# jscanvic/Scale-Equivariant-Imaging

Measured on AMD Instinct MI355X. Metric: training images/sec (256x256 crops), proposed-loss deblur, higher is better.
Workload: dtype bf16; 1 GPU; BASELINE configs[1]: deblurring Gaussian_R2 noise=5, proposed loss (SURE + scale-EI), 256x256 pairs cropped to 48 in Loss.forward, ConvolutionalModel hidden=32 scales=5; parameters=645063043, batch_per_gpu=32, global_batch=32, parallelism=dp1

## Files before the change

scale-equivariant-imaging_amd/csrc/gemm_bf16nt.hip:

```cpp
#include "sei_common.h"

namespace {

typedef __attribute__((address_space(3))) void lds_void;
typedef __attribute__((address_space(1))) const void glb_void;

constexpr int BK = 64;
constexpr int ROW_BYTES = 128;
constexpr int NWAVES = 8, NT = 512;

__device__ __attribute__((aligned(16))) unsigned short g_zero_chunk[8] = {0, 0, 0, 0, 0, 0, 0, 0};

struct NtArgs {
    const unsigned short *A, *B;
    float *D32;
    unsigned short *D16;
    int M, N, K, lda, ldb;
    int epilogue;
    const float *bias, *R1, *R2;
    unsigned short *D2_16;
    int splitk, k_per_split;
    int tiles_m, tiles_n;
    int tiles_per_xcd, band;
    const unsigned short *A2, *B2;
// ... 52 lines not shown

__device__ __forceinline__ void stage_piece_rmajor(const unsigned short *__restrict__ G,
                                                   const unsigned short *__restrict__ G2, int k_seg, int ld, int o0,
                                                   int o_lim, int k0, int k_lim, char *lds_tile, int q, int lane) {
    const int row = 4 * q + (lane >> 4);
    const int ch = (lane & 15) ^ swz_rmajor(row);
    const int k = k0 + row, o = o0 + 8 * ch;
    const unsigned short *rowp = k < k_seg ? G + (size_t)k * ld : G2 + (size_t)(k - k_seg) * ld;
    const unsigned short *src = (k < k_lim && o < o_lim) ? rowp + o : g_zero_chunk;
    dma16_lane(src, lds_tile + q * 1024);
}
__device__ __forceinline__ void stage_tile_rmajor(const unsigned short *__restrict__ G,
                                                  const unsigned short *__restrict__ G2, int k_seg, int ld, int o0,
                                                  int o_lim, int k0, int k_lim, char *lds_tile, int wave, int lane) {
#pragma unroll
    for (int q0 = 0; q0 < 16; q0 += NWAVES)
        stage_piece_rmajor(G, G2, k_seg, ld, o0, o_lim, k0, k_lim, lds_tile, q0 + wave, lane);
}

__device__ __forceinline__ bf16x8 frag_rmajor(const char *tile, int s, int lane, int c0) {
    const int g = lane >> 4, i16 = lane & 15, q = i16 >> 2, p = i16 & 3;
    const int col0 = c0 + 16 * (g & 1);
    const int row = 16 * s + 8 * (g >> 1) + q;
    const int chunk = (col0 >> 3) + (p >> 1);
    auto addr = [&](int r) {
        return (__attribute__((address_space(3))) v4s *)(tile + 256 * r + 16 * (chunk ^ swz_rmajor(r)) + 8 * (p & 1));
    };
    const v4s lo = __builtin_amdgcn_ds_read_tr16_b64_v4i16(addr(row));
    const v4s hi = __builtin_amdgcn_ds_read_tr16_b64_v4i16(addr(row + 4));
    const v8s both = __builtin_shufflevector(lo, hi, 0, 1, 2, 3, 4, 5, 6, 7);
    return __builtin_bit_cast(bf16x8, both);
}

template <int TM, int TN, int WM, int WN, int NSTAGE>
constexpr bool patch_fits() {
    return (NSTAGE * (32 * TM * WM + 32 * TN * WN) * ROW_BYTES) / (32 * TN * WN * 4) >= 32 * TM;
}

template <int TM, int TN, int WM, int WN, bool ARM, bool BRM, int NSTAGE = 2, int ROWEPI = 0>
__global__ __launch_bounds__(NT, (NSTAGE == 1 ? 3 : 1)) void gemm_bf16nt_kernel(NtArgs g) {
    static_assert(WM * WN == NWAVES, "8 waves per workgroup");
    constexpr int BM = 32 * TM * WM, BN = 32 * TN * WN;
    static_assert(!ARM || BM == 128, "a reduction-major A tile is 64 x 128");
    static_assert(!BRM || BN % 128 == 0, "a reduction-major B tile is BN/128 images of 64 k-rows x 128 columns");
    constexpr int STAGE = (BM + BN) * ROW_BYTES;
    __shared__ __attribute__((aligned(1024))) char smem[NSTAGE * STAGE];

    const int lane = threadIdx.x & 63;
    const int wave = __builtin_amdgcn_readfirstlane(threadIdx.x >> 6);
    const int wm = wave / WN, wn = wave % WN;
    const int li = lane & 31, lh = lane >> 5;

    int bid = blockIdx.x;
    const unsigned short *Bp = g.B, *B2p = g.B2;
    float *D32p = g.D32;
    if constexpr (ROWEPI == 3) {
        const int per = gridDim.x / g.batch, bt = bid / per;
        bid -= bt * per;
        const ptrdiff_t shift = (ptrdiff_t)g.batch_row[bt] * g.ldb;
        Bp += shift;
        B2p += shift;
        D32p += (size_t)bt * g.batch_ld;
    }
    int zs, ord;
    if (g.tiles_per_xcd == 0) {
        const int ntile = g.tiles_m * g.tiles_n;
        zs = bid / ntile;
        ord = bid - zs * ntile;
    } else {
        const int per_split = 8 * g.tiles_per_xcd;
        zs = bid / per_split;
        bid -= zs * per_split;
        ord = (bid & 7) * g.tiles_per_xcd + (bid >> 3);
        if ((bid >> 3) >= g.tiles_per_xcd || ord >= g.tiles_m * g.tiles_n) return;
    }
    int tm_i, tn_i;
    {
        const int band_tiles = g.tiles_m * g.band;
        const int b = ord / band_tiles, r = ord - b * band_tiles;
        const int width = min(g.band, g.tiles_n - b * g.band);
        tm_i = r / width;
        tn_i = b * g.band + (r - tm_i * width);
    }
    const int m0 = tm_i * BM, n0 = tn_i * BN;
    const int M = g.M, N = g.N, K = g.K;
    const int k_begin = zs * g.k_per_split;
    const int k_end = min(K, k_begin + g.k_per_split);

    f32x16 acc[TM][TN];
#pragma unroll
    for (int i = 0; i < TM; ++i)
#pragma unroll
        for (int j = 0; j < TN; ++j)
#pragma unroll
            for (int r = 0; r < 16; ++r) acc[i][j][r] = 0.f;

    constexpr bool PREFETCH_AUX = false;
    const int epi = g.epilogue;
    const bool lead = zs == 0;
    const bool split = g.splitk > 1;
    const float *aux1p = nullptr, *aux2p = nullptr;
    if (epi == SEI_EPI_BIAS_RES && (!split || lead)) { aux1p = g.R1; aux2p = g.R2; }
    else if (epi == SEI_EPI_BIAS_SCALE_RES) aux1p = g.R2;
    else if (epi == SEI_EPI_MUL_DGELU) aux1p = g.R1;
    else if (epi == SEI_EPI_ACCUM && !split) aux1p = D32p;
    float a1[TM][TN][16], a2[TM][TN][16];
    auto gather_aux = [&](int i, int j) {
        const int col = n0 + wn * (32 * TN) + 32 * j + li;
        const int row_base = m0 + wm * (32 * TM) + 32 * i + 4 * lh;
#pragma unroll
        for (int r = 0; r < 16; ++r) {
            const int row = row_base + (r & 3) + 8 * (r >> 2);
            const bool ok = col < N && row < M;
            const size_t o = (size_t)row * N + col;
            a1[i][j][r] = (ok && aux1p) ? aux1p[o] : 0.f;
            a2[i][j][r] = (ok && aux2p) ? aux2p[o] : 0.f;
        }
    };
    if constexpr (PREFETCH_AUX) {
        if (aux1p) {
#pragma unroll
            for (int i = 0; i < TM; ++i)
#pragma unroll
                for (int j = 0; j < TN; ++j) gather_aux(i, j);
        } else {
#pragma unroll
            for (int i = 0; i < TM; ++i)
#pragma unroll
                for (int j = 0; j < TN; ++j)
#pragma unroll
                    for (int r = 0; r < 16; ++r) a1[i][j][r] = a2[i][j][r] = 0.f;
        }
    }

    constexpr int NPA = ARM ? 2 : (BM + 63) / 64, NPB = BN / 64;
    static_assert(BN % 64 == 0, "whole pieces per wave");
    unsigned off_a[NPA], off_b[NPB];
#pragma unroll
    for (int e = 0; e < NPA; ++e) {
        const int q = wave + NWAVES * e;
        if constexpr (ARM) {
            const int row = 4 * q + (lane >> 4), ch = (lane & 15) ^ swz_rmajor(row);
            off_a[e] = (unsigned)row * (unsigned)g.lda * 2u + 2u * (unsigned)min(8 * ch, M - 8 - m0);
        } else {
            const int row = 8 * q + (lane >> 3), c = (lane & 7) ^ ((row >> 1) & 7);
            off_a[e] = (unsigned)min(row, M - 1 - m0) * (unsigned)g.lda * 2u + 16u * c;
        }
    }
#pragma unroll
    for (int e = 0; e < NPB; ++e) {
        const int q = wave + NWAVES * e;
        if constexpr (BRM) {
            const int im = q >> 4, qq = q & 15;
            const int row = 4 * qq + (lane >> 4), ch = (lane & 15) ^ swz_rmajor(row);
            off_b[e] = (unsigned)row * (unsigned)g.ldb * 2u +
                       2u * (unsigned)max(min(128 * im + 8 * ch, N - 8 - n0), 0);
        } else {
            const int row = 8 * q + (lane >> 3), c = (lane & 7) ^ ((row >> 1) & 7);
            off_b[e] = (unsigned)min(row, N - 1 - n0) * (unsigned)g.ldb * 2u + 16u * c;
        }
    }
    auto rm_base = [&](const unsigned short *X1, const unsigned short *X2, int ld, int o0, int k0) -> const char * {
        if (k0 + BK <= g.k_seg && k0 + BK <= k_end) return reinterpret_cast<const char *>(X1 + (size_t)k0 * ld + o0);
        if (k0 >= g.k_seg && k0 + BK <= k_end) return reinterpret_cast<const char *>(X2 + (size_t)(k0 - g.k_seg) * ld + o0);
        return nullptr;
    };
    auto stage = [&](int k0, char *dst) {
        const char *ab, *bb;
        if constexpr (ARM) ab = rm_base(g.A, g.A2, g.lda, m0, k0);
        else if (g.conv_cin > 0) {
            const int tap = k0 / g.conv_cin;
            ab = reinterpret_cast<const char *>(g.A + ((ptrdiff_t)m0 + g.conv_off[tap]) * (ptrdiff_t)g.lda +
                                                (k0 - tap * g.conv_cin));
        }
        else ab = k0 + BK <= k_end ? reinterpret_cast<const char *>(g.A + (size_t)m0 * g.lda + k0) : nullptr;
        if (ab) {
#pragma unroll
            for (int e = 0; e < NPA; ++e)
                if (ARM || wave + NWAVES * e < BM / 8)
                    dma16_base(ab, off_a[e], dst + (wave + NWAVES * e) * 1024);
        } else {
            if constexpr (ARM) stage_tile_rmajor(g.A, g.A2, g.k_seg, g.lda, m0, M, k0, k_end, dst, wave, lane);
            else stage_tile<BM>(g.A, g.lda, m0, M, k0, k_end, dst, wave, lane);
        }
        if constexpr (BRM) bb = rm_base(Bp, B2p, g.ldb, n0, k0);
        else bb = k0 + BK <= k_end ? reinterpret_cast<const char *>(Bp + (size_t)n0 * g.ldb + k0) : nullptr;
        if (bb) {
#pragma unroll
            for (int e = 0; e < NPB; ++e)
                dma16_base(bb, off_b[e], dst + BM * ROW_BYTES + (wave + NWAVES * e) * 1024);
        } else if constexpr (BRM) {
#pragma unroll
            for (int im = 0; im < BN / 128; ++im)
                stage_tile_rmajor(Bp, B2p, g.k_seg, g.ldb, n0 + 128 * im, N, k0, k_end,
                                  dst + BM * ROW_BYTES + im * 16384, wave, lane);
        } else {
            stage_tile<BN>(Bp, g.ldb, n0, N, k0, k_end, dst + BM * ROW_BYTES, wave, lane);
        }
    };
    const int sw = (li >> 1) & 7;
    const int a_off = (wm * 32 * TM + li) * ROW_BYTES;
    const int b_off = BM * ROW_BYTES + (wn * 32 * TN + li) * ROW_BYTES;

    auto compute = [&](const char *now) {
#pragma unroll
        for (int s = 0; s < BK / 16; ++s) {
            const int pc = ((2 * s + lh) ^ sw) * 16;
            bf16x8 a[TM], b[TN];
#pragma unroll
            for (int i = 0; i < TM; ++i) {
                if constexpr (ARM) a[i] = frag_rmajor(now, s, lane, wm * 32 * TM + 32 * i);
                else a[i] = *reinterpret_cast<const bf16x8 *>(now + a_off + i * 32 * ROW_BYTES + pc);
            }
#pragma unroll
            for (int j = 0; j < TN; ++j) {
                if constexpr (BRM) {
                    const int c0 = wn * 32 * TN + 32 * j;
                    b[j] = frag_rmajor(now + BM * ROW_BYTES + (c0 >> 7) * 16384, s, lane, c0 & 127);
                }
                else b[j] = *reinterpret_cast<const bf16x8 *>(now + b_off + j * 32 * ROW_BYTES + pc);
            }
#pragma unroll
            for (int i = 0; i < TM; ++i)
#pragma unroll
                for (int j = 0; j < TN; ++j)
                    acc[i][j] = __builtin_amdgcn_mfma_f32_32x32x16_bf16(a[i], b[j], acc[i][j], 0, 0, 0);
        }
    };

    if constexpr (NSTAGE == 1) {
        for (int k0 = k_begin; k0 < k_end; k0 += BK) {
            stage(k0, smem);
            asm volatile("s_waitcnt vmcnt(0)" ::: "memory");
            __syncthreads();
            compute(smem);
            __syncthreads();
        }
    } else if constexpr (NSTAGE == 2) {
        stage(k_begin, smem);
        asm volatile("s_waitcnt vmcnt(0)" ::: "memory");
        __syncthreads();
        int cur = 0;
        for (int k0 = k_begin; k0 < k_end; k0 += BK) {
            if (k0 + BK < k_end) stage(k0 + BK, smem + (cur ^ 1) * STAGE);
            compute(smem + cur * STAGE);
            asm volatile("s_waitcnt vmcnt(0)" ::: "memory");
            __syncthreads();
            cur ^= 1;
        }
    } else {
        constexpr int PER = (BM + BN) / 64;
        static_assert((BM + BN) % 64 == 0, "uniform DMA count per wave");
        const int nt = (k_end - k_begin + BK - 1) / BK;
#pragma unroll
        for (int t = 0; t < NSTAGE - 1; ++t)
            if (t < nt) stage(k_begin + t * BK, smem + t * STAGE);
        int slot = 0;
        for (int t = 0; t < nt; ++t) {
            if (t + NSTAGE - 2 < nt) sei_wait_vmcnt<(NSTAGE - 2) * PER>();
            else sei_wait_vmcnt<0>();
            __builtin_amdgcn_s_barrier();
            const int tn = t + NSTAGE - 1;
            if (tn < nt) {
                int ns = slot + NSTAGE - 1;
                if (ns >= NSTAGE) ns -= NSTAGE;
                stage(k_begin + tn * BK, smem + ns * STAGE);
            }
            compute(smem + slot * STAGE);
            if (++slot == NSTAGE) slot = 0;
        }
        sei_wait_vmcnt<0>();
    }

    if constexpr (ROWEPI == 2) {
        static_assert(TM == 2 && TN == 1 && WM == 2 && WN == 4, "the row patch below is laid out for the 128 x 128 tile");
        float *patch = reinterpret_cast<float *>(smem);
#pragma unroll
        for (int h = 0; h < 2; ++h) {
            __builtin_amdgcn_s_barrier();
            if (wm == h) {
#pragma unroll
                for (int i = 0; i < TM; ++i)
#pragma unroll
                    for (int r = 0; r < 16; ++r)
                        patch[(32 * i + 4 * lh + (r & 3) + 8 * (r >> 2)) * 128 + 32 * wn + li] = acc[i][0][r];
            }
            __syncthreads();
#pragma unroll
            for (int k = 0; k < 4; ++k) {
                const int idx = threadIdx.x + NT * k, r = idx >> 5, c4 = idx & 31;
                const int row = m0 + 64 * h + r, col = n0 + 4 * c4;
                if (row >= M || col >= N) continue;
                const float4 v = *reinterpret_cast<const float4 *>(patch + r * 128 + 4 * c4);
                uint2 w;
                w.x = sei_pack2_bf16(v.x, v.y);
                w.y = sei_pack2_bf16(v.z, v.w);
                *reinterpret_cast<uint2 *>(g.D16 + (size_t)row * N + col) = w;
            }
        }
        return;
    }
    if constexpr (ROWEPI == 1) {
        static_assert(TM == 2 && TN == 1 && WM == 2 && WN == 4, "the row patch below is laid out for the 128 x 128 tile");
        const float beta1 = g.adam_h[0], beta2 = g.adam_h[1], eps = g.adam_h[2], wd = g.adam_h[3];
        const float step_size = g.adam_h[4], inv_bc2_sqrt = g.adam_h[5];
        float *patch = reinterpret_cast<float *>(smem);
#pragma unroll
        for (int h = 0; h < 2; ++h) {
            __builtin_amdgcn_s_barrier();
            if (wm == h) {
#pragma unroll
                for (int i = 0; i < TM; ++i)
#pragma unroll
                    for (int r = 0; r < 16; ++r)
                        patch[(32 * i + 4 * lh + (r & 3) + 8 * (r >> 2)) * 128 + 32 * wn + li] = acc[i][0][r];
            }
            __syncthreads();
#pragma unroll 1
          for (int kk = 0; kk < 4; kk += 2) {
            float4 gq[2], pq[2], mq[2], vq[2];
            size_t off[2];
            bool ok[2];
#pragma unroll
            for (int k = 0; k < 2; ++k) {
                const int idx = threadIdx.x + NT * (kk + k), r = idx >> 5, c4 = idx & 31;
                const int row = m0 + 64 * h + r, col = n0 + 4 * c4;
                ok[k] = row < M && col < N;
                off[k] = ok[k] ? (size_t)row * N + col : 0;
                gq[k] = *reinterpret_cast<const float4 *>(patch + r * 128 + 4 * c4);
                pq[k] = nt_load4(g.adam_p + off[k]);
                mq[k] = nt_load4(g.adam_m + off[k]);
                vq[k] = nt_load4(g.adam_v + off[k]);
            }
#pragma unroll
            for (int k = 0; k < 2; ++k) {
                if (!ok[k]) continue;
                float4 o;
                o.x = sei_adam_element(pq[k].x, gq[k].x, mq[k].x, vq[k].x, beta1, beta2, eps, wd, step_size, inv_bc2_sqrt);
                o.y = sei_adam_element(pq[k].y, gq[k].y, mq[k].y, vq[k].y, beta1, beta2, eps, wd, step_size, inv_bc2_sqrt);
                o.z = sei_adam_element(pq[k].z, gq[k].z, mq[k].z, vq[k].z, beta1, beta2, eps, wd, step_size, inv_bc2_sqrt);
                o.w = sei_adam_element(pq[k].w, gq[k].w, mq[k].w, vq[k].w, beta1, beta2, eps, wd, step_size, inv_bc2_sqrt);
                nt_store4(g.adam_m + off[k], mq[k]);
                nt_store4(g.adam_v + off[k], vq[k]);
                nt_store4(g.adam_p + off[k], o);
                if (g.adam_p16) {
                    uint2 w;
                    w.x = sei_pack2_bf16(o.x, o.y);
                    w.y = sei_pack2_bf16(o.z, o.w);
                    u32x2 t;
                    t.x = w.x; t.y = w.y;
                    __builtin_nontemporal_store(t, reinterpret_cast<u32x2 *>(g.adam_p16 + off[k]));
                }
            }
          }
        }
        return;
    }

    if constexpr ((ROWEPI == 4 || ROWEPI == 5) && patch_fits<TM, TN, WM, WN, NSTAGE>()) {
        constexpr int ROWS_WM = 32 * TM;
        constexpr int LDS_ROWS = (NSTAGE * STAGE) / (BN * 4);
        constexpr int GW = LDS_ROWS >= WM * ROWS_WM ? WM : (LDS_ROWS >= 2 * ROWS_WM && WM >= 2 ? 2 : 1);
        static_assert(LDS_ROWS >= ROWS_WM && WM % GW == 0, "one wave row of the tile fits the operand stages");
        constexpr int RP = GW * ROWS_WM, QPR = BN / 4, TOTAL = RP * QPR;
        float *patch = reinterpret_cast<float *>(smem);
        const bool to_bf16_only = g.D16 != nullptr && D32p == nullptr;
#pragma unroll 1
        for (int pass = 0; pass < WM / GW; ++pass) {
            __builtin_amdgcn_s_barrier();
            if (wm / GW == pass) {
#pragma unroll
                for (int i = 0; i < TM; ++i)
#pragma unroll
                    for (int j = 0; j < TN; ++j)
#pragma unroll
                        for (int r = 0; r < 16; ++r)
                            patch[((wm % GW) * ROWS_WM + 32 * i + 4 * lh + (r & 3) + 8 * (r >> 2)) * BN + wn * (32 * TN) +
                                  32 * j + li] = acc[i][j][r];
            }
            __syncthreads();
            constexpr int U = NSTAGE == 1 ? 1 : 2;
#pragma unroll 1
            for (int base = threadIdx.x; base < TOTAL; base += U * NT) {
                float4 v[U], r1[U], r2[U];
                size_t off[U];
                int rowi[U];
                bool ok[U];
#pragma unroll
                for (int u = 0; u < U; ++u) {
                    const int idx = base + u * NT;
                    const int r = idx / QPR, c4 = idx - r * QPR;
                    int row = m0 + pass * RP + r;
                    const int col = n0 + 4 * c4;
                    ok[u] = idx < TOTAL && row < M && col < N;
                    if constexpr (ROWEPI == 5) {
                        const int Wp = g.unpad_W + 2, HWp = (g.unpad_H + 2) * Wp;
                        const int b = row / HWp, rem = row - b * HWp, yy = rem / Wp, xx = rem - yy * Wp;
                        ok[u] = ok[u] && yy >= 1 && yy <= g.unpad_H && xx >= 1 && xx <= g.unpad_W;
                        row = (b * g.unpad_H + yy - 1) * g.unpad_W + xx - 1;
                    }
                    off[u] = ok[u] ? (size_t)row * N + col : 0;
                    rowi[u] = ok[u] ? row : 0;
                    v[u] = *reinterpret_cast<const float4 *>(patch + (idx < TOTAL ? r * BN + 4 * c4 : 0));
                    r1[u] = r2[u] = make_float4(0.f, 0.f, 0.f, 0.f);
                    if (epi == SEI_EPI_BIAS || epi == SEI_EPI_BIAS_GELU || epi == SEI_EPI_BIAS_RES ||
                        epi == SEI_EPI_BIAS_ROWSCALE || epi == SEI_EPI_BIAS_SCALE_RES) {
                        const int cb = ok[u] ? col : 0;
                        float4 b = make_float4(g.bias[cb], g.bias[cb + 1], g.bias[cb + 2], g.bias[cb + 3]);
                        if (epi == SEI_EPI_BIAS_ROWSCALE) {
                            const float sc = g.R1[rowi[u]];
                            b.x *= sc; b.y *= sc; b.z *= sc; b.w *= sc;
                        }
                        v[u].x += b.x; v[u].y += b.y; v[u].z += b.z; v[u].w += b.w;
                    }
                    if (epi == SEI_EPI_BIAS_RES || epi == SEI_EPI_MUL_DGELU)
                        r1[u] = *reinterpret_cast<const float4 *>(g.R1 + off[u]);
                    else if (epi == SEI_EPI_ACCUM) r1[u] = *reinterpret_cast<const float4 *>(D32p + off[u]);
                    if (epi == SEI_EPI_BIAS_SCALE_RES || (epi == SEI_EPI_BIAS_RES && g.R2))
                        r2[u] = *reinterpret_cast<const float4 *>(g.R2 + off[u]);
                }
#pragma unroll
                for (int u = 0; u < U; ++u) {
                    if (!ok[u]) continue;
                    float4 o = v[u];
                    if (epi == SEI_EPI_MUL_DGELU) {
                        if (to_bf16_only) {
                            o.x *= sei_dgelu_bf16out(r1[u].x); o.y *= sei_dgelu_bf16out(r1[u].y);
                            o.z *= sei_dgelu_bf16out(r1[u].z); o.w *= sei_dgelu_bf16out(r1[u].w);
                        } else {
                            o.x *= sei_dgelu(r1[u].x); o.y *= sei_dgelu(r1[u].y);
                            o.z *= sei_dgelu(r1[u].z); o.w *= sei_dgelu(r1[u].w);
                        }
                    } else if (epi == SEI_EPI_BIAS_SCALE_RES) {
                        const float sc = g.R1[rowi[u]];
                        o.x = fmaf(o.x, sc, r2[u].x); o.y = fmaf(o.y, sc, r2[u].y);
                        o.z = fmaf(o.z, sc, r2[u].z); o.w = fmaf(o.w, sc, r2[u].w);
                    } else {
                        if (ROWEPI == 5 && g.unpad_act) {
                            o.x = o.x > 0.f ? o.x : 0.01f * o.x; o.y = o.y > 0.f ? o.y : 0.01f * o.y;
                            o.z = o.z > 0.f ? o.z : 0.01f * o.z; o.w = o.w > 0.f ? o.w : 0.01f * o.w;
                        }
                        o.x += r1[u].x + r2[u].x; o.y += r1[u].y + r2[u].y;
                        o.z += r1[u].z + r2[u].z; o.w += r1[u].w + r2[u].w;
                    }
                    if (epi == SEI_EPI_BIAS_GELU) {
                        uint2 w;
                        w.x = (unsigned)sei_f2bf(sei_gelu_bf16out(o.x)) | ((unsigned)sei_f2bf(sei_gelu_bf16out(o.y)) << 16);
                        w.y = (unsigned)sei_f2bf(sei_gelu_bf16out(o.z)) | ((unsigned)sei_f2bf(sei_gelu_bf16out(o.w)) << 16);
                        *reinterpret_cast<uint2 *>(g.D2_16 + off[u]) = w;
                    }
                    if (D32p) *reinterpret_cast<float4 *>(D32p + off[u]) = o;
                    if (g.D16) {
                        uint2 w;
                        w.x = sei_pack2_bf16(o.x, o.y);
                        w.y = sei_pack2_bf16(o.z, o.w);
                        *reinterpret_cast<uint2 *>(g.D16 + off[u]) = w;
                    }
                }
            }
        }
        return;
    }

#pragma unroll
    for (int i = 0; i < TM; ++i) {
#pragma unroll
        for (int j = 0; j < TN; ++j) {
            const int col = n0 + wn * (32 * TN) + 32 * j + li;
            const bool col_ok = col < N;
            const int row_base = m0 + wm * (32 * TM) + 32 * i + 4 * lh;
            float bias = (col_ok && (!split || lead) &&
                          (epi == SEI_EPI_BIAS || epi == SEI_EPI_BIAS_GELU || epi == SEI_EPI_BIAS_RES ||
                           epi == SEI_EPI_BIAS_ROWSCALE || epi == SEI_EPI_BIAS_SCALE_RES))
                             ? g.bias[col] : 0.f;
            if constexpr (!PREFETCH_AUX) gather_aux(i, j);
            if (epi == SEI_EPI_BIAS_ROWSCALE) {
#pragma unroll
                for (int r = 0; r < 16; ++r) {
                    const int row = row_base + (r & 3) + 8 * (r >> 2);
                    a1[i][j][r] = row < M ? bias * g.R1[row] : 0.f;
                }
                bias = 0.f;
            }
#pragma unroll
            for (int r = 0; r < 16; ++r) {
                const int row = row_base + (r & 3) + 8 * (r >> 2);
                if (!col_ok || row >= M) continue;
                const size_t o = (size_t)row * N + col;
                float v = acc[i][j][r] + bias;
                if (split) {
                    atomicAdd(D32p + o, v + a1[i][j][r] + a2[i][j][r]);
                    continue;
                }
                if (epi == SEI_EPI_MUL_DGELU)
                    v *= (g.D16 && !D32p) ? sei_dgelu_bf16out(a1[i][j][r]) : sei_dgelu(a1[i][j][r]);
                else if (epi == SEI_EPI_BIAS_SCALE_RES) v = fmaf(v, g.R1[row], a1[i][j][r]);
                else v += a1[i][j][r] + a2[i][j][r];
                if (epi == SEI_EPI_BIAS_GELU) g.D2_16[o] = sei_f2bf(sei_gelu_bf16out(v));
                if (D32p) D32p[o] = v;
                if (g.D16) g.D16[o] = sei_f2bf(v);
            }
        }
    }
}

__global__ __launch_bounds__(256) void zero_fill_kernel(float *__restrict__ p, size_t n) {
    const size_t stride = (size_t)gridDim.x * blockDim.x;
    const size_t n4 = n / 4;
    for (size_t i = (size_t)blockIdx.x * blockDim.x + threadIdx.x; i < n4; i += stride)
        reinterpret_cast<float4 *>(p)[i] = make_float4(0.f, 0.f, 0.f, 0.f);
    for (size_t i = n4 * 4 + (size_t)blockIdx.x * blockDim.x + threadIdx.x; i < n; i += stride) p[i] = 0.f;
}

#ifdef SEI_TUNING
int g_tuning_tile = 0, g_tuning_band = 0, g_tuning_splitk = 0;
#include "gemm_bf16pp.h"
#endif
#include "gemm_bf16pq.h"

template <int TM, int TN, int WM, int WN, bool ARM = false, bool BRM = false, int NSTAGE = 2, int ROWEPI = 0>
int launch_nt(NtArgs &g, hipStream_t s) {
    constexpr int BM = 32 * TM * WM, BN = 32 * TN * WN;
    g.tiles_m = (int)sei_ceil_div(g.M, BM);
    g.tiles_n = (int)sei_ceil_div(g.N, BN);
    const size_t tiles = (size_t)g.tiles_m * g.tiles_n;
    const size_t nbatch = g.batch > 1 ? (size_t)g.batch : 1;
    SEI_REQUIRE(tiles * nbatch < ((size_t)1 << 27));
    {
        constexpr size_t STAGE_BYTES = NSTAGE * (size_t)(BM + BN) * ROW_BYTES;
        const double conc = 32.0 * (STAGE_BYTES <= 40 * 1024 ? 3 : (STAGE_BYTES <= 80 * 1024 ? 2 : 1));
        int band = g.force_band > 0 ? g.force_band : (int)(sqrt(conc * BM / BN) + 0.5);
        if (band < 1) band = 1;
        if (band > g.tiles_n) band = g.tiles_n;
        g.band = band;
        g.tiles_per_xcd = tiles < 64 ? 0 : (int)sei_ceil_div(tiles, 8);
    }
    g.splitk = 1;
    g.k_per_split = g.K;
    const bool splittable = (g.epilogue == SEI_EPI_NONE || g.epilogue == SEI_EPI_BIAS ||
                             g.epilogue == SEI_EPI_BIAS_RES || g.epilogue == SEI_EPI_ACCUM) && !g.unpad_W;
    if ((ROWEPI == 0 || ROWEPI == 3) && splittable && g.D32 && !g.D16 && g.K >= 8 * BK) {
        constexpr size_t STAGE_BYTES = NSTAGE * (size_t)(BM + BN) * ROW_BYTES;
        const size_t slots = 256 * (STAGE_BYTES <= 40 * 1024 ? 3 : (STAGE_BYTES <= 80 * 1024 ? 2 : 1));
        const size_t ktiles = sei_ceil_div(g.K, BK);
        const size_t max_sk = ktiles / 4 < 256 ? ktiles / 4 : 256;
        const double overhead = 6.0 + (g.epilogue == SEI_EPI_ACCUM ? 0.0 : 2.0);
        const double split_cost = g.epilogue == SEI_EPI_ACCUM ? 2.0 : 32.0;
        double best = 1e30;
        size_t best_sk = 1;
        for (size_t sk = 1; sk <= max_sk; ++sk) {
            const double rounds = (double)sei_ceil_div(tiles * nbatch * sk, slots);
            const double cost = rounds * ((double)sei_ceil_div(ktiles, sk) + overhead + (sk > 1 ? split_cost : 0.0));
            if (cost < best * 0.97) {
                best = cost;
                best_sk = sk;
            }
        }
#ifdef SEI_TUNING
        if (g_tuning_splitk > 0) best_sk = (size_t)g_tuning_splitk < ktiles ? (size_t)g_tuning_splitk : ktiles;
#endif
        if (best_sk > 1) {
            g.k_per_split = (int)(sei_ceil_div(ktiles, best_sk) * BK);
            g.splitk = (int)sei_ceil_div(g.K, g.k_per_split);
        }
    }
    if (g.plan) {
        *g.plan = (1ull << 48) | ((unsigned long long)BM << 32) | ((unsigned long long)BN << 16) | (unsigned)g.splitk;
        return SEI_OK;
    }
    if (g.splitk > 1 && g.epilogue != SEI_EPI_ACCUM) {
        if (nbatch > 1) return SEI_ERR_BAD_ARG;
        const size_t n = (size_t)g.M * g.N;
        size_t zg = sei_ceil_div(n / 4 + 1, 256);
        if (zg > 2048) zg = 2048;
        if ((reinterpret_cast<uintptr_t>(g.D32) & 15) != 0) return SEI_ERR_BAD_ARG;
        hipLaunchKernelGGL(zero_fill_kernel, dim3((unsigned)zg), dim3(256), 0, s, g.D32, n);
    }
    const size_t per_split = g.tiles_per_xcd ? 8 * (size_t)g.tiles_per_xcd : tiles;
    if constexpr (ROWEPI == 0 && patch_fits<TM, TN, WM, WN, NSTAGE>()) {
        const auto al = [](const void *p, uintptr_t m) { return (reinterpret_cast<uintptr_t>(p) & m) == 0; };
        const bool r1_rows = g.epilogue == SEI_EPI_BIAS_ROWSCALE || g.epilogue == SEI_EPI_BIAS_SCALE_RES;
        if (g.splitk == 1 && g.N % 4 == 0 && al(g.D32, 15) && al(g.D16, 7) && al(g.D2_16, 7) && (r1_rows || al(g.R1, 15)) &&
            al(g.R2, 15) && !g.force_band) {
            if constexpr (!ARM && !BRM && NSTAGE == 2) {
                if (g.unpad_W) {
                    hipLaunchKernelGGL((gemm_bf16nt_kernel<TM, TN, WM, WN, ARM, BRM, NSTAGE, 5>), dim3((unsigned)per_split),
                                       dim3(NT), 0, s, g);
                    return sei_launch_status();
                }
            }
            hipLaunchKernelGGL((gemm_bf16nt_kernel<TM, TN, WM, WN, ARM, BRM, NSTAGE, 4>), dim3((unsigned)per_split), dim3(NT),
                               0, s, g);
            return sei_launch_status();
        }
    }
    if (g.unpad_W) return SEI_ERR_BAD_ARG;
    hipLaunchKernelGGL((gemm_bf16nt_kernel<TM, TN, WM, WN, ARM, BRM, NSTAGE, ROWEPI>),
                       dim3((unsigned)(per_split * g.splitk * nbatch)),
                       dim3(NT), 0, s, g);
    return sei_launch_status();
}

}

#ifdef SEI_TUNING
extern "C" int sei_debug_set_nt_tile(int code) {
    if (code >= 1000) {
        g_tuning_splitk = code - 1000;
        return SEI_OK;
    }
    if (code >= 100) {
        g_tuning_band = code - 100;
        return SEI_OK;
    }
    g_tuning_tile = code;
    return SEI_OK;
}
#endif

int pq_choose(const NtArgs &g, bool would_split) {
    const int M = g.M, N = g.N, K = g.K;
    const int rf = M % 288 == 0 ? 9 : ((M % 256 == 0 || M >= 4096) ? 8 : 0);
    if (g.force_tile != 0 || !rf || K < 32 || N < 128 || !pq_eligible(g)) return 0;
    const size_t tm = sei_ceil_div(M, 32 * rf);
    const size_t t4 = N >= 256 ? tm * sei_ceil_div(N, 256) : 0, t2 = tm * sei_ceil_div(N, 128);
    auto fills = [](size_t t) { return (double)t / (double)(sei_ceil_div(t, 256) * 256) >= 0.8; };
    if (K < 128 && (would_split || N > 128)) return 0;
    if (N < 512 && would_split) return 0;
    if (t4 >= 192 && fills(t4)) return 10 * rf + 4;
    if (t2 >= 192 && t4 < 192 && fills(t2)) return 10 * rf + 2;
    if (would_split) {
        if (K < 8192 || N < 2048 || (M < 2304 && N < 8192)) return 0;
        return 10 * rf + ((t4 >= 96 || (t4 >= 64 && N >= 8192)) ? 4 : 2);
    }
    if (t2 >= 128 && t4 < 192) return 10 * rf + 2;
    return 0;
}

int pq_choose_slabs(NtArgs &g, bool would_split) {
    const int M = g.M, N = g.N, K = g.K;
    if (!g.ws || !would_split || g.epilogue == SEI_EPI_ACCUM || g.force_tile != 0 || g.force_splitk != 0) return 0;
    if (K < 2048 || K % BK != 0 || N < 512 || !pq_eligible(g)) return 0;
    const int rf = M % 288 == 0 ? 9 : ((M % 256 == 0 || M >= 4096) ? 8 : 0);
    if (!rf) return 0;
    const size_t tm = sei_ceil_div(M, 32 * rf), kt = (size_t)K / BK;
    const bool from_hbm = (double)N * (double)K * 2.0 >= 128.0 * 1048576.0;
    double best = 1e30;
    int best_nf = 0, best_sk = 1;
    for (int nf = 2; nf <= 4; nf += 2) {
        const size_t tiles = tm * sei_ceil_div(N, 64 * nf);
        const double c = nf == 2 ? (from_hbm ? 1.05 : 0.95) : (from_hbm ? 1.75 : 1.5);
        const double o = nf == 2 ? 10.0 : 16.0, e0 = nf == 2 ? 5.0 : 8.0, e1 = nf == 2 ? 3.0 : 5.0;
        const size_t slab = (size_t)32 * rf * 64 * nf * 4;
        for (size_t sk = 1; sk <= 16 && sk * 4 <= kt; ++sk) {
            if (sk > 1 && (tiles > 4096 || 16384 + tiles * sk * slab > g.ws_bytes || sk * slab >= ((size_t)1 << 31))) break;
            const double rounds = (double)sei_ceil_div(tiles * sk, 256);
            const double cost = rounds * ((double)sei_ceil_div(kt, sk) * c + o + (sk > 1 ? e0 + e1 * (double)(sk - 1) : 0.0));
// ... 433 lines not shown
```

Baseline: 2733 images/s.

## Stage full tile in LDS and software-pipeline Adam state loads in fused epilogue

The fused Adam epilogue now writes the whole 128x128 accumulator tile to LDS in one pass instead of two half-tile passes, which removes one barrier round. It also issues the param, m and v loads for the first groups before the LDS write and keeps a rolling prefetch of two groups ahead, so global-load latency overlaps with the LDS staging and the Adam math. In exchange it uses more registers for the prefetch buffers (three buffers of three float4 pairs), which can lower occupancy, and it relies on the operand stages being large enough to hold the full float tile.

Measured after the change: 2742 images/s, median of 3. Within noise of the previous version (+0.3%).

```diff
diff --git a/scale-equivariant-imaging_amd/csrc/gemm_bf16nt.hip b/scale-equivariant-imaging_amd/csrc/gemm_bf16nt.hip
--- a/scale-equivariant-imaging_amd/csrc/gemm_bf16nt.hip
+++ b/scale-equivariant-imaging_amd/csrc/gemm_bf16nt.hip
@@ -378,57 +378,62 @@
     }
     if constexpr (ROWEPI == 1) {
         static_assert(TM == 2 && TN == 1 && WM == 2 && WN == 4, "the row patch below is laid out for the 128 x 128 tile");
+        static_assert(NSTAGE * STAGE >= BM * BN * 4, "the whole tile as floats inside the operand stages");
+        constexpr int G = 2, NGRP = 8 / G, AHEAD = 2, NBUF = AHEAD + 1;
         const float beta1 = g.adam_h[0], beta2 = g.adam_h[1], eps = g.adam_h[2], wd = g.adam_h[3];
         const float step_size = g.adam_h[4], inv_bc2_sqrt = g.adam_h[5];
         float *patch = reinterpret_cast<float *>(smem);
-#pragma unroll
-        for (int h = 0; h < 2; ++h) {
-            __builtin_amdgcn_s_barrier();
-            if (wm == h) {
-#pragma unroll
-                for (int i = 0; i < TM; ++i)
-#pragma unroll
-                    for (int r = 0; r < 16; ++r)
-                        patch[(32 * i + 4 * lh + (r & 3) + 8 * (r >> 2)) * 128 + 32 * wn + li] = acc[i][0][r];
-            }
-            __syncthreads();
-#pragma unroll 1
-          for (int kk = 0; kk < 4; kk += 2) {
-            float4 gq[2], pq[2], mq[2], vq[2];
-            size_t off[2];
-            bool ok[2];
-#pragma unroll
-            for (int k = 0; k < 2; ++k) {
-                const int idx = threadIdx.x + NT * (kk + k), r = idx >> 5, c4 = idx & 31;
-                const int row = m0 + 64 * h + r, col = n0 + 4 * c4;
-                ok[k] = row < M && col < N;
-                off[k] = ok[k] ? (size_t)row * N + col : 0;
-                gq[k] = *reinterpret_cast<const float4 *>(patch + r * 128 + 4 * c4);
-                pq[k] = nt_load4(g.adam_p + off[k]);
-                mq[k] = nt_load4(g.adam_m + off[k]);
-                vq[k] = nt_load4(g.adam_v + off[k]);
-            }
-#pragma unroll
-            for (int k = 0; k < 2; ++k) {
-                if (!ok[k]) continue;
+        const int pr = threadIdx.x >> 5, pc = 4 * (threadIdx.x & 31);
+        const int row0 = m0 + pr, col = n0 + pc;
+        const bool col_ok = col < N;
+        auto quad_ok = [&](int j) { return col_ok && row0 + 16 * j < M; };
+        auto quad_off = [&](int j) { return quad_ok(j) ? (size_t)(row0 + 16 * j) * N + col : (size_t)0; };
+        float4 pq[NBUF][G], mq[NBUF][G], vq[NBUF][G];
+        auto load_group = [&](int grp) {
+#pragma unroll
+            for (int k = 0; k < G; ++k) {
+                const size_t off = quad_off(G * grp + k);
+                pq[grp % NBUF][k] = nt_load4(g.adam_p + off);
+                mq[grp % NBUF][k] = nt_load4(g.adam_m + off);
+                vq[grp % NBUF][k] = nt_load4(g.adam_v + off);
+            }
+        };
+#pragma unroll
+        for (int grp = 0; grp < AHEAD; ++grp) load_group(grp);
+        __builtin_amdgcn_s_barrier();
+#pragma unroll
+        for (int i = 0; i < TM; ++i)
+#pragma unroll
+            for (int r = 0; r < 16; ++r)
+                patch[(64 * wm + 32 * i + 4 * lh + (r & 3) + 8 * (r >> 2)) * 128 + 32 * wn + li] = acc[i][0][r];
+        __syncthreads();
+#pragma unroll
+        for (int grp = 0; grp < NGRP; ++grp) {
+            if (grp + AHEAD < NGRP) load_group(grp + AHEAD);
+#pragma unroll
+            for (int k = 0; k < G; ++k) {
+                const int j = G * grp + k;
+                if (!quad_ok(j)) continue;
+                const size_t off = quad_off(j);
+                const float4 gq = *reinterpret_cast<const float4 *>(patch + (pr + 16 * j) * 128 + pc);
+                float4 &p = pq[grp % NBUF][k], &m = mq[grp % NBUF][k], &v = vq[grp % NBUF][k];
                 float4 o;
-                o.x = sei_adam_element(pq[k].x, gq[k].x, mq[k].x, vq[k].x, beta1, beta2, eps, wd, step_size, inv_bc2_sqrt);
-                o.y = sei_adam_element(pq[k].y, gq[k].y, mq[k].y, vq[k].y, beta1, beta2, eps, wd, step_size, inv_bc2_sqrt);
-                o.z = sei_adam_element(pq[k].z, gq[k].z, mq[k].z, vq[k].z, beta1, beta2, eps, wd, step_size, inv_bc2_sqrt);
-                o.w = sei_adam_element(pq[k].w, gq[k].w, mq[k].w, vq[k].w, beta1, beta2, eps, wd, step_size, inv_bc2_sqrt);
-                nt_store4(g.adam_m + off[k], mq[k]);
-                nt_store4(g.adam_v + off[k], vq[k]);
-                nt_store4(g.adam_p + off[k], o);
+                o.x = sei_adam_element(p.x, gq.x, m.x, v.x, beta1, beta2, eps, wd, step_size, inv_bc2_sqrt);
+                o.y = sei_adam_element(p.y, gq.y, m.y, v.y, beta1, beta2, eps, wd, step_size, inv_bc2_sqrt);
+                o.z = sei_adam_element(p.z, gq.z, m.z, v.z, beta1, beta2, eps, wd, step_size, inv_bc2_sqrt);
+                o.w = sei_adam_element(p.w, gq.w, m.w, v.w, beta1, beta2, eps, wd, step_size, inv_bc2_sqrt);
+                nt_store4(g.adam_m + off, m);
+                nt_store4(g.adam_v + off, v);
+                nt_store4(g.adam_p + off, o);
                 if (g.adam_p16) {
                     uint2 w;
                     w.x = sei_pack2_bf16(o.x, o.y);
                     w.y = sei_pack2_bf16(o.z, o.w);
                     u32x2 t;
                     t.x = w.x; t.y = w.y;
-                    __builtin_nontemporal_store(t, reinterpret_cast<u32x2 *>(g.adam_p16 + off[k]));
+                    __builtin_nontemporal_store(t, reinterpret_cast<u32x2 *>(g.adam_p16 + off));
                 }
             }
-          }
         }
         return;
     }
```
